# hermanjakobsen/robotic-ultrasound-imaging

Hardware: AMD Instinct MI355X
Metric: env-steps/sec (whole node) at 4096 envs/GPU, random-action rollout (higher is better)
Workload: dtype f32

## Files before the change

### robotic-ultrasound-imaging_amd/csrc/usim_api.hip

```cpp
#include <hip/hip_runtime.h>
#include <cstdio>
#include <cstdlib>
#include <cstring>
#include <string>
#include <vector>
#include <new>

#include "../../include/usim.h"
#include "usim_device.h"
#include "usim_robot.h"
#include "usim_setup.h"
#include "usim_checkpoint.h"
#include "usim_kernels.hip"
#include "usim_snapshot.h"


using namespace usim;

enum class Launch : int { STEP, MULTI, ACTS, RESET };
constexpr Launch launch_kind(bool reset, int nsub, int substeps, const float* act) {
    return reset ? Launch::RESET : nsub > 1 ? (act ? Launch::ACTS : Launch::MULTI) : substeps > 1 ? Launch::MULTI : Launch::STEP;
}

using StepKernel = void (*)(const DevModel, const DevCfg, float*, int, int, const DevIO, int, long long);
using SplitKernel = void (*)(const DevModel*, const DevCfg*, float*, int, int, const DevIO, int, long long);
struct Kernel { StepKernel step; SplitKernel split; int epb, nt, lds_words; };
struct Row { Mapping map; bool warm; Launch launch; Kernel k; };

template <Launch L> constexpr Row full_row() {
    static_assert(L == Launch::STEP || L == Launch::RESET, "the full torso runs one step per launch");
    StepKernel f = nullptr;
    if constexpr (L == Launch::STEP) f = usim_step_kernel<2, 64, 0>;
    else f = usim_step_kernel<2, 64, 1>;
    return {Mapping::FULL, false, L, {f, nullptr, FULL_EPB, FULL_NT, FULL_LDS_WORDS}};
}
template <int TORSO, int OCC, bool WARM, Launch L> constexpr Row wave_row() {
    static_assert((TORSO == 1 || (TORSO == 0 && OCC == 2 && !WARM)) && (L != Launch::RESET || OCC == 2), "RIGID16, SOFT16_W1, SOFT16_W2; resets with the budget of two waves per SIMD");
    StepKernel f = nullptr;
    if constexpr (L == Launch::STEP) f = usim_step16_kernel<TORSO, OCC, 0, false, WARM>;
    else if constexpr (L == Launch::MULTI) f = usim_step16_kernel<TORSO, OCC, 0, true, WARM>;
    else if constexpr (L == Launch::ACTS) f = usim_step16_acts_kernel<TORSO, OCC, WARM>;
    else f = usim_step16_kernel<TORSO, OCC, 1, false, WARM>;
    return {TORSO == 0 ? Mapping::RIGID16 : OCC == 1 ? Mapping::SOFT16_W1 : Mapping::SOFT16_W2, WARM, L, {f, nullptr, 16, 256, arm_lds_base<TORSO, 0, 16>() + ARM_LDS_WORDS}};
}
template <int G, bool WARM, Launch L> constexpr Row split_row() {
    static_assert((G == 16 || G == 8) && L != Launch::RESET, "SPLIT16, SPLIT8; they reset with SOFT16_W2's kernel");
    SplitKernel f = nullptr;
    if constexpr (L == Launch::STEP) f = usim_step32_kernel<false, G, WARM>;
    else if constexpr (L == Launch::MULTI) f = usim_step32_kernel<true, G, WARM>;
    else f = usim_step32_acts_kernel<G, WARM>;
    return {G == 16 ? Mapping::SPLIT16 : Mapping::SPLIT8, WARM, L, {nullptr, f, (64 / G) * SPLIT_WPR, 128 * SPLIT_WPR, arm_lds_base<1, 1, G>() + ARM_LDS_WORDS}};
}

constexpr Row kRows[] = {
    wave_row<0, 2, false, Launch::ACTS>(),
    wave_row<1, 1, true, Launch::ACTS>(), wave_row<1, 1, false, Launch::ACTS>(), wave_row<1, 2, true, Launch::ACTS>(), wave_row<1, 2, false, Launch::ACTS>(),
    split_row<16, true, Launch::ACTS>(), split_row<16, false, Launch::ACTS>(), split_row<8, true, Launch::ACTS>(), split_row<8, false, Launch::ACTS>(),

    wave_row<1, 2, true, Launch::RESET>(),
    wave_row<1, 1, true, Launch::MULTI>(), wave_row<1, 1, true, Launch::STEP>(), wave_row<1, 2, true, Launch::MULTI>(), wave_row<1, 2, true, Launch::STEP>(),
    split_row<16, true, Launch::MULTI>(), split_row<16, true, Launch::STEP>(), split_row<8, true, Launch::MULTI>(), split_row<8, true, Launch::STEP>(),

    full_row<Launch::RESET>(), full_row<Launch::STEP>(),
    wave_row<0, 2, false, Launch::MULTI>(), wave_row<0, 2, false, Launch::STEP>(), wave_row<0, 2, false, Launch::RESET>(),
    wave_row<1, 1, false, Launch::MULTI>(), wave_row<1, 1, false, Launch::STEP>(), wave_row<1, 2, false, Launch::MULTI>(), wave_row<1, 2, false, Launch::STEP>(),
    wave_row<1, 2, false, Launch::RESET>(),
    split_row<16, false, Launch::MULTI>(), split_row<16, false, Launch::STEP>(), split_row<8, false, Launch::MULTI>(), split_row<8, false, Launch::STEP>(),
};

constexpr int find_row(Mapping m, bool warm, Launch l) {
    if (m == Mapping::FULL && l != Launch::RESET) l = Launch::STEP;
    if (soft_torso(m) && l == Launch::RESET) m = Mapping::SOFT16_W2;
    warm = warm && soft_torso(m);
    int at = -1, hits = 0;
    for (int i = 0; i < (int)(sizeof kRows / sizeof kRows[0]); ++i)
        if (kRows[i].map == m && kRows[i].warm == warm && kRows[i].launch == l) { at = i; ++hits; }
    return hits == 1 ? at : -1;
}
constexpr bool table_sound() {
    for (const Row& r : kRows) if (r.k.lds_words * (int)sizeof(float) > 160 * 1024 || r.k.nt > 1024 || r.k.epb < 1 || (r.k.step == nullptr) == (r.k.split == nullptr)) return false;
    for (int m = 0; m <= (int)Mapping::SPLIT8; ++m) for (int w = 0; w < 2; ++w) for (int l = 0; l <= (int)Launch::RESET; ++l) if (find_row((Mapping)m, w != 0, (Launch)l) < 0) return false;
    return true;
}
static_assert(table_sound(), "every row within 160 KB of LDS and 1024 threads; every (mapping, warm, launch) has exactly one row");
static const Kernel& kernel_of(Mapping m, bool warm, Launch l) { return kRows[find_row(m, warm, l)].k; }

struct usim_handle {
    usim_config cfg;
    Mapping map = Mapping::RIGID16;
    StateLayout L{};
    int device = 0, adim = 6;
    DevModel M;
    DevCfg C;
    float* state = nullptr;
    float* d_tables = nullptr;
    void* d_consts = nullptr;
    const DevModel* d_M = nullptr; const DevCfg* d_C = nullptr;
    hipEvent_t ev0 = nullptr, ev1 = nullptr;
    static constexpr int RF_RING = 8;
    hipEvent_t rf0[RF_RING] = {}, rf1[RF_RING] = {};
    bool rf_live[RF_RING] = {};
    int rf_next = 0;
    double rf_total_ms = 0.0;
    long long rf_count = 0;
// ... 429 lines not shown
```

### robotic-ultrasound-imaging_amd/csrc/usim_step16.h

```cpp
#pragma once
#include <type_traits>

namespace usim {

template <int N, class F>
DI void static_for(F&& f) {
    if constexpr (N > 0) { static_for<N - 1>(f); f(std::integral_constant<int, N - 1>{}); }
}

template <int CTRL>
DI float dpp0(float v) { return __int_as_float(__builtin_amdgcn_update_dpp(0, __float_as_int(v), CTRL, 0xf, 0xf, true)); }
template <int G> DI int glane() { return (int)(threadIdx.x & (G - 1)); }
template <int G, int K> DI float rbc(float v) {
    if constexpr (G == 16) return dpp0<0x150 + K>(v);
    else {
        const int iv = __float_as_int(v);
        const int t = __builtin_amdgcn_update_dpp(iv, iv, 0x150 + K, 0xf, 0x3, false);
        return __int_as_float(__builtin_amdgcn_update_dpp(t, iv, 0x150 + 8 + K, 0xf, 0xc, false));
    }
}
template <int G, int D> DI float rshr0(float v) {
    const float t = dpp0<0x110 + D>(v);
    if constexpr (G == 16) return t; else return (glane<G>() < D) ? 0.f : t;
}
// ... 110 lines not shown
DI void fk16(const float* at, const float q, f3& X, f3& Y, f3& Z, f3& P) {
    float s, c;
    sincos_(q, s, c);
    const f3 f0 = mk(at[AT_RFIX], at[AT_RFIX + 1], at[AT_RFIX + 2]), f1 = mk(at[AT_RFIX + 3], at[AT_RFIX + 4], at[AT_RFIX + 5]);
    X = f0 * c + f1 * s; Y = f1 * c - f0 * s; Z = mk(at[AT_RFIX + 6], at[AT_RFIX + 7], at[AT_RFIX + 8]);
    P = mk(at[AT_LPOS], at[AT_LPOS + 1], at[AT_LPOS + 2]);
    static_for<3>([&](auto Dc) {
        constexpr int D = 1 << decltype(Dc)::value;
        const f3 LX = mk(rshr<G, D>(X.x, 1.f), rshr<G, D>(X.y, 0.f), rshr<G, D>(X.z, 0.f));
        const f3 LY = mk(rshr<G, D>(Y.x, 0.f), rshr<G, D>(Y.y, 1.f), rshr<G, D>(Y.z, 0.f));
        const f3 LZ = mk(rshr<G, D>(Z.x, 0.f), rshr<G, D>(Z.y, 0.f), rshr<G, D>(Z.z, 1.f));
        const f3 LP = mk(rshr0<G, D>(P.x), rshr0<G, D>(P.y), rshr0<G, D>(P.z));
        const f3 nX = LX * X.x + LY * X.y + LZ * X.z, nY = LX * Y.x + LY * Y.y + LZ * Y.z, nZ = LX * Z.x + LY * Z.y + LZ * Z.z;
        P = LP + LX * P.x + LY * P.y + LZ * P.z;
        X = nX; Y = nY; Z = nZ;
    });
}

DI void jacobian_rows(float* xl, const int gl, const float* Jc, float* Jr) {
    if (gl < 8) {
#pragma unroll
        for (int a = 0; a < 6; ++a) xl[a * 8 + gl] = Jc[a];
    }
    group_sync();
    int arow = (gl & 7) - ((gl & 4) ? 1 : 0);
    arow = arow > 5 ? 5 : arow;
    const float4 j0 = *reinterpret_cast<const float4*>(&xl[arow * 8]), j1 = *reinterpret_cast<const float4*>(&xl[arow * 8 + 4]);
    Jr[0] = j0.x; Jr[1] = j0.y; Jr[2] = j0.z; Jr[3] = j0.w; Jr[4] = j1.x; Jr[5] = j1.y; Jr[6] = j1.z; Jr[7] = j1.w;
}

template <int G>
DI float solve6_task(float* A, float b, const int gl) {
    static_for<6>([&](auto Kc) {
        constexpr int k = decltype(Kc)::value;
        constexpr int lk = TASK_LANE[k];
        const float g = (A[k] - (gl == lk ? 1.f : 0.f)) * rcp_(rbc<G, lk>(A[k]));
#pragma unroll
        for (int c = k + 1; c < 6; ++c) A[c] = fmaf(-g, rbc<G, lk>(A[c]), A[c]);
        b = fmaf(-g, rbc<G, lk>(b), b);
    });
    return b;
}

constexpr int X16_WORDS = 64;
constexpr int X16_RIGID_STRIDE = 84;

constexpr int SPLIT_WPR = 4;
constexpr int MB_POSE = X16_WORDS;
constexpr int MB_OP = MB_POSE + 12;
constexpr int MB_W = MB_OP + 64;
constexpr int MB_Q = MB_W + 16;
constexpr int MB_GOAL = MB_Q + 100;
constexpr int MB_ACT = MB_GOAL + 12;
constexpr int X2_STRIDE = MB_ACT + 8;
template <int G> constexpr int x2_base() { return TB_WORDS + (64 * SPLIT_WPR / G) * GE_STRIDE; }
static_assert(x2_base<16>() % 4 == 0 && x2_base<8>() % 4 == 0 && X2_STRIDE % 4 == 0 && MB_OP % 4 == 0 && MB_W % 4 == 0 && MB_ACT % 4 == 0, "mailbox block: 16-byte accesses");
static_assert((x2_base<8>() + 32 * X2_STRIDE) * 4 <= 160 * 1024, "split kernel with 8-lane groups: LDS of a CU");
template <int G> constexpr int arm_cull_rounds() { return G == 16 ? 0 : 7; }
template <int ROLE, int G, bool RES> constexpr bool lattice_ahead() { return ROLE != 0 && G == 16 && RES; }

#if defined(USIM_TSTAMP) || defined(USIM_TSTAMP_NOWAIT)
#define USIM_BAR() do { __syncthreads(); ++nbar; } while (0)
#else
#define USIM_BAR() __syncthreads()
#endif


constexpr int ARM_LDS_WORDS = A16_LANES * AT_STRIDE;
template <int TORSO, int ROLE, int G> constexpr int arm_lds_base();
template <int NE, class WR = NoWarm>
struct Carry {
    float dqj, qdj, q0j;
    Episode ep;
    float s[NE], sd[NE];
    WR wr;
};

template <int TORSO, int ROLE, int G> constexpr int arm_lds_base() {
    return ROLE != 0 ? x2_base<G>() + (64 * SPLIT_WPR / G) * X2_STRIDE : (TORSO ? SOFT16_LDS_WORDS : 16 * X16_RIGID_STRIDE);
}
static_assert((arm_lds_base<1, 1, 8>() + ARM_LDS_WORDS) * 4 <= 160 * 1024 && arm_lds_base<1, 1, 8>() % 4 == 0 && arm_lds_base<1, 1, 16>() % 4 == 0 && arm_lds_base<1, 0, 16>() % 4 == 0
              && arm_lds_base<0, 0, 16>() % 4 == 0, "arm table behind the LDS blocks of every 16-lane kernel");

template <int NT, int G, bool RES, class WR>
DI void lattice_pass(float* lds, const DevModel& M, const DevCfg& C, float* __restrict__ st, const int n, const int npad, const DevIO& io,
                     const bool first_pass, const int sub, const bool more, int& nbar, Carry<(N_TOP + G - 1) / G, WR>& cy) {
    constexpr bool WARM = !std::is_same<WR, NoWarm>::value;
    constexpr int WPR = SPLIT_WPR, EPW = 64 / G, EPB = WPR * EPW;
    constexpr unsigned GMASK = (G == 16) ? 0xffffu : 0xffu;
    constexpr int NE = (N_TOP + G - 1) / G;
    constexpr bool LA = lattice_ahead<2, G, RES>();
    const int lane = threadIdx.x & 63, wave = (threadIdx.x >> 6) & (WPR - 1);
    const bool fresh = !RES || first_pass;
    const int gl = lane & (G - 1), ge = lane / G;
    const int gbase = lane - gl;
    const int eb = wave * EPW + ge;
    unsigned long long* const dbg = io.dbg;
    const int env = blockIdx.x * EPB + eb;
    const bool valid = env < n;
    const bool store = valid && gl == 0;
    const int ei = valid ? env : n - 1;
#define LAT(w) st[(size_t)F_LAT * npad + (size_t)ei * LAT_ENV_WORDS + (w)]
#define EB(off) lds[TB_WORDS + eb * GE_STRIDE + (off)]
    float* const warm_rows = st + warm_index(io.bank_row0, npad, (size_t)ei);
    int mbo = x2_base<G>() + eb * X2_STRIDE;
    asm volatile("" : "+v"(mbo));

    float* const xl = &lds[mbo];
    float* const goal_lds = xl + MB_GOAL;
    float at[AT_STRIDE];
    {
        constexpr int ARM_LDS = arm_lds_base<1, 2, G>();
        const float4* ap = fresh ? reinterpret_cast<const float4*>(M.tables + TB_ARM + gl * AT_STRIDE) : reinterpret_cast<const float4*>(lds + ARM_LDS + gl * AT_STRIDE);
        if (fresh) {
#pragma unroll
            for (int v = 0; v < AT_STRIDE / 4; ++v) { const float4 x = ap[v]; at[4 * v] = x.x; at[4 * v + 1] = x.y; at[4 * v + 2] = x.z; at[4 * v + 3] = x.w; }
        } else {
            const float4* lp = reinterpret_cast<const float4*>(lds + ARM_LDS + gl * AT_STRIDE);
#pragma unroll
            for (int v = 0; v < AT_STRIDE / 4; ++v) { const float4 x = lp[v]; at[4 * v] = x.x; at[4 * v + 1] = x.y; at[4 * v + 2] = x.z; at[4 * v + 3] = x.w; }
        }
    }
    const float* const sp = st + scalar_index(0, (size_t)ei);
    const bool jlane = at[AT_JOINT] != 0.f;
    const int jl = jlane ? gl : NJ - 1;
    float &dqj = cy.dqj, &qdj = cy.qdj, &q0j = cy.q0j;
    Episode& E = cy.ep;
    f3 &ts = E.ts, &te = E.te;
    float &u0 = E.u0, &vbar = E.vbar, &fzbar = E.fzbar, &fzprev = E.fzprev, &dfz = E.dfz, &kst = E.kst, &kdmp = E.kdmp, &mu = E.mu, &epret = E.epret;
    int &t = E.t, &touched = E.touched, &episode = E.episode, &status = E.status;
    float (&s_pre)[NE] = cy.s, (&sd_pre)[NE] = cy.sd;
    auto adopt = [&](const float4 nx) {
        kst = nx.x; kdmp = nx.y; mu = nx.z; t = 0;
#pragma unroll
        for (int i = 0; i < NE; ++i) { s_pre[i] = 0.f; sd_pre[i] = 0.f; }
        warm_clear(cy.wr);
    };
    if (fresh) {
        dqj = sp[F_Q + jl]; qdj = sp[F_QD + jl]; q0j = sp[F_Q0 + jl];
        float sv[20];
        {
            const float4* s4 = reinterpret_cast<const float4*>(sp + 20);
#pragma unroll
            for (int v = 0; v < 5; ++v) { const float4 x = s4[v]; sv[4 * v] = x.x; sv[4 * v + 1] = x.y; sv[4 * v + 2] = x.z; sv[4 * v + 3] = x.w; }
        }
#define SV(f) sv[(f) - 20]
        ts = mk(SV(F_TS), SV(F_TS + 1), SV(F_TS + 2)); te = mk(SV(F_TE), SV(F_TE + 1), SV(F_TE + 2));
        u0 = SV(F_U0); vbar = SV(F_VBAR); fzbar = SV(F_FZBAR); fzprev = SV(F_FZPREV); dfz = SV(F_DFZ);
        kst = SV(F_KST); kdmp = SV(F_KDMP); mu = SV(F_MU); epret = SV(F_EPRET);
        t = __float_as_int(SV(F_T)); touched = __float_as_int(SV(F_TOUCH)); episode = __float_as_int(SV(F_EPISODE)); status = __float_as_int(SV(F_STATUS));
#undef SV
#pragma unroll
        for (int i = 0; i < NE; ++i) {
            const int e = gl + i * G;
            s_pre[i] = 0.f; sd_pre[i] = 0.f;
            if (e < N_TOP) { s_pre[i] = LAT(LAT_S + e); sd_pre[i] = LAT(LAT_SD + e); }
        }
        if constexpr (WARM) warm_load(warm_rows, gl, cy.wr);
    } else if constexpr (RES && !LA) {
        const float4 nx = *reinterpret_cast<const float4*>(&lds[mbo + MB_W]);
        if (nx.w != 0.f) adopt(nx);
    }
    if (!jlane) { dqj = 0.f; qdj = 0.f; q0j = 0.f; }
    float qj = q0j + dqj;
    if (first_pass) {
// ... 136 lines not shown
    RSTAMP(6);
#if defined(USIM_TSTAMP) || defined(USIM_TSTAMP_NOWAIT)
    if (more && dbg && blockIdx.x == 0 && (threadIdx.x & (64 * WPR - 1)) == 0) dbg[62] = __builtin_readcyclecounter();
#endif
    {
        float acc_e[NE];
#pragma unroll
        for (int i = 0; i < NE; ++i) { const int e = gl + i * G; acc_e[i] = (e < N_TOP) ? EB(GE_A + e) : 0.f; }
#pragma unroll
        for (int k = 0; k < MAXC; ++k) {
#pragma unroll
            for (int i = 0; i < NE; ++i) {
                const int e = (gl + i * G < N_TOP) ? gl + i * G : N_TOP - 1;
                acc_e[i] = fmaf(lds[TB_LINV + e * LROW + cel[k]], gf[k], acc_e[i]);
            }
        }
#pragma unroll
        for (int i = 0; i < NE; ++i) {
            const int e = gl + i * G;
            if (e >= N_TOP) continue;
            const float sdn = sd_pre[i] + dt * acc_e[i];
            const float sn = s_pre[i] + dt * sdn;
            if (valid) { LAT(LAT_SD + e) = sdn; LAT(LAT_S + e) = sn; }
            if constexpr (RES) { sd_pre[i] = sdn; s_pre[i] = sn; EB(GE_S + e) = sn; }
        }
        if constexpr (WARM) { if (valid) warm_store(warm_rows, gl, cy.wr); }
    }
    RSTAMP(7);
    if (!LA || !more) USIM_BAR();
    RSTAMP(8);
#undef RSTAMP
#undef XSTAMP
#undef LAT
#undef EB
}

template <int TORSO, int MODE, int ROLE, int NT, int G = 16, bool RES = false, class WR = NoWarm, bool AHEAD = false>
DI void step16_one(float* lds, const DevModel& M, const DevCfg& C, float* __restrict__ st, const int n, const int npad, const DevIO& io, const int flags, const long long rstep,
                   const bool first_pass, const int sub, const bool more, int& nbar, Carry<TORSO ? (N_TOP + G - 1) / G : 1, WR>& cy) {
    static_assert(ROLE != 2, "the lattice / contact wave of the split kernel runs lattice_pass");
    static_assert(!AHEAD || (ROLE == 1 && RES), "action drawn ahead: the arm wave of a resident split launch");
    constexpr bool WARM = !std::is_same<WR, NoWarm>::value;
    static_assert(!WARM || (TORSO == 1 && ROLE == 0) || (TORSO == 1 && MODE == 0), "warm start: the soft-torso kernels");
    constexpr int WPR = (ROLE != 0) ? SPLIT_WPR : 4;
    constexpr int EPW = 64 / G, EPB = WPR * EPW;
    static_assert(!RES || MODE == 0, "resident state: step launches only");
    constexpr int X2_BASE = x2_base<G>();
    constexpr unsigned GMASK = (G == 16) ? 0xffffu : 0xffu;
    static_assert(G == 16 || (TORSO == 1 && MODE == 0 && ROLE != 0), "8-lane groups: the split soft-torso step only");
    constexpr int NE = TORSO ? (N_TOP + G - 1) / G : 1;
    static_assert(ROLE == 0 || (TORSO == 1 && MODE == 0), "the split kernel is the soft-torso step");
    const int lane = threadIdx.x & 63, wave = (threadIdx.x >> 6) & (WPR - 1);
    constexpr bool LA = lattice_ahead<ROLE, G, RES>();
    const bool fresh = !RES || first_pass;
    const int gl = lane & (G - 1), ge = lane / G;
    const int gbase = lane - gl;
    const int eb = wave * EPW + ge;
    const bool auto_reset = (flags & LF_AUTO_RESET) != 0;
    unsigned long long* const dbg = io.dbg;
    const bool refill = (MODE == 1) && io.refill != 0;
    const int item_cnt = refill ? io.count[0] : 1;
    const int item_first = refill ? (int)blockIdx.x * EPB : 0;
    for (int item0 = item_first; item0 < item_cnt; item0 += refill ? (int)gridDim.x * EPB : 1) {
    int env = blockIdx.x * EPB + eb;
    bool valid = env < n;
    int item_ep = 0;
    if (refill) {
        valid = item0 + eb < item_cnt;
        const int2 it = valid ? io.items[item0 + eb] : make_int2(0, 0);
        env = it.x; item_ep = it.y;
    }
    const bool store = valid && gl == 0;
    const int ei = valid ? env : (refill ? 0 : n - 1);
#define LAT(w) st[(size_t)F_LAT * npad + (size_t)ei * LAT_ENV_WORDS + (w)]
#define EB(off) lds[TB_WORDS + eb * GE_STRIDE + (off)]
    float* const warm_rows = st + warm_index(io.bank_row0, npad, (size_t)ei);
    int mbo = X2_BASE + eb * X2_STRIDE;
    if constexpr (ROLE != 0) asm volatile("" : "+v"(mbo));
    float* const xl = (ROLE != 0) ? &lds[mbo]
                                  : (TORSO ? &lds[TB_WORDS + eb * GE_STRIDE + GE_WS] : &lds[eb * X16_RIGID_STRIDE]);
    static_assert(GE_WS + X16_WORDS <= GE_STRIDE, "transpose scratch overlays the wrench records");
    constexpr int GOAL_OFF = (ROLE != 0) ? MB_GOAL : (TORSO ? GE_CG + (MAXCAND + 1) * CG_WORDS - GE_WS : X16_WORDS);
    static_assert(GE_CG + (MAXCAND + 1) * CG_WORDS + 12 <= GE_STRIDE && X16_WORDS + 12 <= X16_RIGID_STRIDE, "room for the goal");
    float* const goal_lds = xl + GOAL_OFF;

    USIM_STAMP(dbg, 0);
    if constexpr (ROLE == 1) { if (dbg && blockIdx.x == 0 && threadIdx.x == 0) dbg[20] = __builtin_readcyclecounter(); }

    float at[AT_STRIDE];
    {
        constexpr int ARM_LDS = arm_lds_base<TORSO, ROLE, G>();
        const float4* ap = fresh ? reinterpret_cast<const float4*>(M.tables + TB_ARM + gl * AT_STRIDE) : reinterpret_cast<const float4*>(lds + ARM_LDS + gl * AT_STRIDE);
        if (fresh) {
#pragma unroll
            for (int v = 0; v < AT_STRIDE / 4; ++v) { const float4 x = ap[v]; at[4 * v] = x.x; at[4 * v + 1] = x.y; at[4 * v + 2] = x.z; at[4 * v + 3] = x.w; }
            if constexpr (RES) {
                if (lane < G) {
#pragma unroll
                    for (int v = 0; v < AT_STRIDE / 4; ++v) reinterpret_cast<float4*>(lds + ARM_LDS + gl * AT_STRIDE)[v] = make_float4(at[4 * v], at[4 * v + 1], at[4 * v + 2], at[4 * v + 3]);
                }
            }
        } else {
            const float4* lp = reinterpret_cast<const float4*>(lds + ARM_LDS + gl * AT_STRIDE);
#pragma unroll
            for (int v = 0; v < AT_STRIDE / 4; ++v) { const float4 x = lp[v]; at[4 * v] = x.x; at[4 * v + 1] = x.y; at[4 * v + 2] = x.z; at[4 * v + 3] = x.w; }
        }
    }
    const float* const sp = st + scalar_index(0, (size_t)ei);
    const bool jlane = at[AT_JOINT] != 0.f;
    const int jl = jlane ? gl : NJ - 1;
    float &dqj = cy.dqj, &qdj = cy.qdj, &q0j = cy.q0j;
    Episode& E = cy.ep;
    f3 &ts = E.ts, &te = E.te;
    float &u0 = E.u0, &vbar = E.vbar, &fzbar = E.fzbar, &fzprev = E.fzprev, &dfz = E.dfz, &kst = E.kst, &kdmp = E.kdmp, &mu = E.mu, &epret = E.epret;
    int &t = E.t, &touched = E.touched, &episode = E.episode, &status = E.status;
    float (&s_pre)[NE] = cy.s, (&sd_pre)[NE] = cy.sd;
    if (fresh) {
        dqj = sp[F_Q + jl]; qdj = sp[F_QD + jl]; q0j = sp[F_Q0 + jl];
        float sv[20];
        {
            const float4* s4 = reinterpret_cast<const float4*>(sp + 20);
#pragma unroll
            for (int v = 0; v < 5; ++v) { const float4 x = s4[v]; sv[4 * v] = x.x; sv[4 * v + 1] = x.y; sv[4 * v + 2] = x.z; sv[4 * v + 3] = x.w; }
        }
#define SV(f) sv[(f) - 20]
        ts = mk(SV(F_TS), SV(F_TS + 1), SV(F_TS + 2)); te = mk(SV(F_TE), SV(F_TE + 1), SV(F_TE + 2));
        u0 = SV(F_U0); vbar = SV(F_VBAR); fzbar = SV(F_FZBAR); fzprev = SV(F_FZPREV); dfz = SV(F_DFZ);
        kst = SV(F_KST); kdmp = SV(F_KDMP); mu = SV(F_MU); epret = SV(F_EPRET);
        t = __float_as_int(SV(F_T)); touched = __float_as_int(SV(F_TOUCH)); episode = __float_as_int(SV(F_EPISODE)); status = __float_as_int(SV(F_STATUS));
#undef SV
#pragma unroll
        for (int i = 0; i < NE; ++i) {
            const int e = gl + i * G;
            s_pre[i] = 0.f; sd_pre[i] = 0.f;
            if (TORSO && MODE == 0 && ROLE == 0 && e < N_TOP) { s_pre[i] = LAT(LAT_S + e); sd_pre[i] = LAT(LAT_SD + e); }
            if (TORSO && MODE == 0 && ROLE == 1 && !LA && e < N_TOP) s_pre[i] = LAT(LAT_S + e);
        }
        if constexpr (WARM && MODE == 0 && ROLE == 0) warm_load(warm_rows, gl, cy.wr);
    } else if constexpr (RES && ROLE == 1 && !LA) {
#pragma unroll
        for (int i = 0; i < NE; ++i) { const int e = gl + i * G; s_pre[i] = (e < N_TOP) ? EB(GE_S + e) : 0.f; }
    }
    if (!jlane) { dqj = 0.f; qdj = 0.f; q0j = 0.f; }
    float qj = q0j + dqj;
// ... 350 lines not shown
    const float alpha_t = row_times_joint<G, NJ>(Jr, qs);
    f3 s_rc, s_wwrc, s_nw, s_arm, s_xso;
    float qe[4], obs[OBS_DIM], pos_err_norm = 0.f, pos_rew = 0.f, ori_err = 0.f, ori_rew = 0.f, vel_rew = 0.f, force_e = 0.f, dforce_e = 0.f;
    f3 xw, tpw;
    auto rot_inertia = [&](f3 v) {
        const f3 l = mk(dot(X, v), dot(Y, v), dot(Z, v));
        const f3 tt = symmul(M.pI7, l);
        return X * tt.x + Y * tt.y + Z * tt.z;
    };
    auto precompute = [&]() {
        s_rc = X * M.pcom7[0] + Y * M.pcom7[1] + Z * M.pcom7[2];
        s_wwrc = cross(w, cross(w, s_rc));
        s_nw = cross(w, rot_inertia(w));
        s_xso = xs - P;
        s_arm = s_rc - s_xso;
        const int tprev = (MODE == 0) ? t - 1 : 0;
        const float up = clampf((float)tprev * inv_h + u0, 0.f, 1.f);
        tpw = ts + (te - ts) * up;
        xw = mk(xs.x + M.base[0], xs.y + M.base[1], xs.z + M.base[2]);
        obs[12] = xw.x - tpw.x; obs[13] = xw.y - tpw.y; obs[14] = xw.z - tpw.z;
        mat2quat_xyzw(sx, sy, sz, qe);
        difference_quat(qe, M.gquat, obs + 15);
        if constexpr (MODE == 0) {
            float pe0 = 90.f * (xw.x - tpw.x), pe1 = 90.f * (xw.y - tpw.y);
            pe0 *= pe0; pe1 *= pe1;
            pos_err_norm = sqrt_(pe0 * pe0 + pe1 * pe1);
            pos_rew = 5.f * exp_(-pos_err_norm);
            const float qc[4] = {qe[3], qe[0], qe[1], qe[2]};
            ori_err = 0.2f * distance_quat_goal(qc, M.ghat, M.geps);
            ori_rew = exp_(-ori_err);
            float ve = 45.f * (vbar - 0.04f); ve *= ve;
            vel_rew = exp_(-ve);
            float fe = 0.7f * (fzbar - 5.f); fe *= fe;
            force_e = 3.f * exp_(-fe);
            float de = 0.01f * dfz; de *= de;
            dforce_e = 2.f * exp_(-de);
        }
    };
    float W[6] = {0, 0, 0, 0, 0, 0};
    int ncon = 0, overflow = 0, con_shell[MAXC];
#pragma unroll
    for (int k = 0; k < MAXC; ++k) con_shell[k] = -1;
    if constexpr (ROLE == 1) {
        if (is_task) {
            const int arow = blk ? 3 + comp : comp;
            float* mbo = xl + MB_OP;
            *reinterpret_cast<float4*>(&mbo[arow * 8]) = make_float4(Li[0], Li[1], Li[2], Li[3]);
            mbo[arow * 8 + 4] = Li[4]; mbo[arow * 8 + 5] = Li[5];
            mbo[48 + arow] = alpha_t; mbo[54 + arow] = v6;
        }
        RSTAMP(3);
        USIM_BAR();
        RSTAMP(4);
        precompute();
        if constexpr (AHEAD) {
            if ((flags & LF_RANDOM_ACT) && more && last_sub) {
                float nxt[7];
                draw_action(rstep + 1, nxt);
                keep_action(nxt);
            }
        }
        RSTAMP(5);
        USIM_BAR();
        RSTAMP(6);
#if defined(USIM_TSTAMP) || defined(USIM_TSTAMP_NOWAIT)
        if (more && dbg && blockIdx.x == 0 && (threadIdx.x & (64 * WPR - 1)) == 0) dbg[63] = __builtin_readcyclecounter();
#endif
        const float4 w0 = *reinterpret_cast<const float4*>(&xl[MB_W]), w1 = *reinterpret_cast<const float4*>(&xl[MB_W + 4]);
        W[0] = w0.x; W[1] = w0.y; W[2] = w0.z; W[3] = w0.w; W[4] = w1.x; W[5] = w1.y;
        ncon = __float_as_int(w1.z); overflow = __float_as_int(w1.w);
        if (io.contacts) {
            const int* tb_shell = reinterpret_cast<const int*>(lds + TB_SHELL);
            const float4 e0 = *reinterpret_cast<const float4*>(&xl[MB_W + 8]), e1 = *reinterpret_cast<const float4*>(&xl[MB_W + 12]);
            const int el[MAXC] = {__float_as_int(e0.x), __float_as_int(e0.y), __float_as_int(e0.z), __float_as_int(e0.w),
                                  __float_as_int(e1.x), __float_as_int(e1.y), __float_as_int(e1.z), __float_as_int(e1.w)};
#pragma unroll
            for (int k = 0; k < MAXC; ++k) { const int sh = tb_shell[el[k]]; con_shell[k] = (k < ncon) ? sh : -1; }
        }
    } else if constexpr (TORSO != 0) {
        const int* tb_shell = reinterpret_cast<const int*>(lds + TB_SHELL);
        float dz, vz, az;
        torso_motion(C, tphys, dz, vz, az);
        lattice_rhs<G, NE>(lds, eb, gl, M, az, kst, kdmp, MODE == 0, s_pre, sd_pre);
        USIM_STAMP(dbg, 5);
        int nc = collide_all<G, NE>(lds, eb, gl, gbase, M, C, MODE == 0, s_pre, dz, xs, sy, sz);
        lattice_solve<G>(lds, eb, gl, gbase);
        contact_overflow<G>(lds, eb, gl, gbase, nc);
        USIM_STAMP(dbg, 7);
        if (nc > MAXC) { overflow = 1; nc = MAXC; }
        ncon = nc;
        group_sync();
        int ncmax = 0;
#pragma unroll
        for (int k = MAXC; k >= 1; --k) if (ncmax == 0 && __any(nc >= k)) ncmax = k;
        float gf[MAXC];
        int cel[MAXC];
#pragma unroll
        for (int k = 0; k < MAXC; ++k) { gf[k] = 0.f; cel[k] = (k < nc) ? __float_as_int(EB(GE_CG + k * CG_WORDS + 6)) : 0; }
        if (ncmax > 0) {
            float alpha[6], vs[6], Lp[21];
            static_for<6>([&](auto Ac) {
                constexpr int a = decltype(Ac)::value;
                alpha[a] = rbc<G, TASK_LANE[a]>(alpha_t); vs[a] = rbc<G, TASK_LANE[a]>(v6);
#pragma unroll
                for (int b = 0; b <= a; ++b) Lp[PK(a, b)] = rbc<G, TASK_LANE[a]>(Li[b]);
            });
            USIM_STAMP(dbg, 8);
            if constexpr (MODE == 0) contact_solve<G, false, false>(lds, eb, gl, M, C, nc, ncmax, cel, Lp, alpha, vs, mu, vz, ContactRows{}, W, gf, dbg, cy.wr);
            else { NoWarm cold; contact_solve<G, false, false>(lds, eb, gl, M, C, nc, ncmax, cel, Lp, alpha, vs, mu, vz, ContactRows{}, W, gf, dbg, cold); }
        } else warm_clear(cy.wr);
        USIM_STAMP(dbg, 11);
        if constexpr (MODE == 1) {
            if (valid && need && !refill) {
                for (int e = gl; e < N_TOP; e += G) { LAT(LAT_S + e) = 0.f; LAT(LAT_SD + e) = 0.f; }
                if constexpr (WARM) warm_rows_clear<G>(warm_rows, gl);
            }
        } else {
            float acc_e[NE];
#pragma unroll
            for (int i = 0; i < NE; ++i) { const int e = gl + i * G; acc_e[i] = (e < N_TOP) ? EB(GE_A + e) : 0.f; }
#pragma unroll
            for (int k = 0; k < MAXC; ++k) {
                if (k < ncmax) {
#pragma unroll
                    for (int i = 0; i < NE; ++i) {
                        const int e = (gl + i * G < N_TOP) ? gl + i * G : N_TOP - 1;
                        acc_e[i] = fmaf(lds[TB_LINV + e * LROW + cel[k]], gf[k], acc_e[i]);
                    }
                }
            }
#pragma unroll
            for (int i = 0; i < NE; ++i) {
                const int e = gl + i * G;
                if (e >= N_TOP) continue;
                const float sdn = sd_pre[i] + dt * acc_e[i];
                const float sn = s_pre[i] + dt * sdn;
                if (valid) { LAT(LAT_SD + e) = sdn; LAT(LAT_S + e) = sn; }
                if constexpr (RES) { sd_pre[i] = sdn; s_pre[i] = sn; }
            }
            if constexpr (WARM) { if (valid) warm_store(warm_rows, gl, cy.wr); }
        }
#pragma unroll
        for (int k = 0; k < MAXC; ++k) con_shell[k] = (k < nc) ? tb_shell[cel[k]] : -1;
    }
    USIM_STAMP(dbg, 12);

    if constexpr (ROLE != 1) precompute();
    float tq[3];
    f3 hv;
    {
        float qacc = qs, aq_t = alpha_t;
        if (TORSO) {
#pragma unroll
            for (int a = 0; a < 6; ++a) { qacc = fmaf(Xm[a], W[a], qacc); aq_t = fmaf(Li[a], W[a], aq_t); }
        }
        float aq[6];
        static_for<6>([&](auto Ac) { constexpr int a = decltype(Ac)::value; aq[a] = rbc<G, TASK_LANE[a]>(aq_t); });
        const f3 alq = mk(aq[3], aq[4], aq[5]);
        const f3 alt = al + alq;
        const f3 a7 = ao + mk(aq[0], aq[1], aq[2]) - cross(alq, s_xso);
        const f3 ac = a7 + cross(alt, s_rc) + s_wwrc;
        const f3 N = rot_inertia(alt) + s_nw;
        const f3 Fp = ac * PROBE_MASS;
        const f3 tw = N + cross(s_arm, Fp) - mk(W[3], W[4], W[5]);
        tq[0] = rbc<G, NJ - 1>(dot(sx, tw)); tq[1] = rbc<G, NJ - 1>(dot(sy, tw)); tq[2] = rbc<G, NJ - 1>(dot(sz, tw));
        USIM_STAMP(dbg, 13);
        hv = mk(0, 0, 0);
        if constexpr (MODE == 0) {
            const float xk = row_times_joint<G, NJ>(Mi, qacc);
            const float rhs = fmaf(-dt * JOINT_DAMP, xk, qacc);
            qdj = fmaf(dt, rhs, qdj); dqj = fmaf(dt, qdj, dqj);
            if (!jlane) { qdj = 0.f; dqj = 0.f; }
            qj = q0j + dqj;
            const float v2_t = row_times_joint<G, NJ>(Jr, qdj);
            float v2[6];
            static_for<6>([&](auto Ac) { constexpr int a = decltype(Ac)::value; v2[a] = rbc<G, TASK_LANE[a]>(v2_t); });
            hv = mk(v2[0], v2[1], v2[2]) + cross(mk(v2[3], v2[4], v2[5]), hand - xs);
        }
    }
    USIM_STAMP(dbg, 14);

    bool done = false;
    {
        if (MODE == 1) fzbar = W[2];
        obs[0] = W[0]; obs[1] = W[1]; obs[2] = W[2];
        obs[3] = tq[0]; obs[4] = tq[1]; obs[5] = tq[2];
        obs[6] = hv.x; obs[7] = hv.y; obs[8] = hv.z;
        obs[9] = fzbar - 5.0f; obs[10] = dfz - 0.0f; obs[11] = vbar - 0.04f;
        if constexpr (MODE == 1) {
            if (overflow) status |= 1;
            if (refill) {
                if (valid && need) {
                    const int sl = ep_t & (BANK_DEPTH - 1);
                    if (jlane) BK(sl, BQ0 + gl) = qj;
                    if (gl == 0) {
                        BK(sl, BTS) = ts.x; BK(sl, BTS + 1) = ts.y; BK(sl, BTS + 2) = ts.z; BK(sl, BTE) = te.x; BK(sl, BTE + 1) = te.y; BK(sl, BTE + 2) = te.z;
                        BK(sl, BU0) = u0; BK(sl, BKST) = kst; BK(sl, BKDMP) = kdmp; BK(sl, BMU) = mu; BK(sl, BFZ) = fzbar;
#pragma unroll
                        for (int a = 0; a < OBS_DIM; ++a) BK(sl, BOBS + a) = obs[a];
                        BKI(sl, BSTATUS) = overflow ? 1 : 0;
                    }
                }
            } else if (store && io.obs && need) {
#pragma unroll
                for (int a = 0; a < OBS_DIM; ++a) io.obs[(size_t)ei * OBS_DIM + a] = obs[a];
            }
        } else if (last_sub) {
        const bool contact = ncon > 0;
        if (contact) touched = 1;
        const float force_rew = contact ? force_e : 0.f, dforce_rew = contact ? dforce_e : 0.f;
        float reward = pos_rew + ori_rew + vel_rew + force_rew + dforce_rew;
        done = t >= C.horizon;
        const float hvn = sqrt_(dot(hv, hv));
        vbar += (hvn - vbar) * rcp_((float)t);
        const float fz = W[2];
        dfz = (fz - fzprev) * rcp_(C.dt_ctrl);
        fzprev = fz;
        fzbar = 0.1f * fz + 0.9f * fzbar;
        const bool jviol = (qj < at[AT_QMIN] + 0.1f) || (qj > at[AT_QMAX] - 0.1f);
        const unsigned jany = (unsigned)(__ballot(jviol) >> gbase) & GMASK;
        if (C.early_term) {
            const bool term = (jany != 0u) || (pos_err_norm > 1.0f) || (contact && ori_err > 0.10f) || (touched && !contact);
            done = done || term;
        }
        epret += reward;
        if (io.log && valid) {
            float* L = io.log + (size_t)ei * LOG_WIDTH;
            if (jlane) L[26 + gl] = qj;
            if (gl == 0) {
                const float upn = clampf((float)t * inv_h + u0, 0.f, 1.f);
                const f3 tpn = ts + (te - ts) * upn;
                L[0] = xw.x; L[1] = xw.y; L[2] = xw.z; L[3] = tpn.x; L[4] = tpn.y; L[5] = tpn.z;
                L[6] = hv.x; L[7] = hv.y; L[8] = hv.z; L[9] = 0.04f; L[10] = vbar;
                L[11] = qe[0]; L[12] = qe[1]; L[13] = qe[2]; L[14] = qe[3];
                L[15] = M.gquat[0]; L[16] = M.gquat[1]; L[17] = M.gquat[2]; L[18] = M.gquat[3];
                L[19] = ori_err * 5.0f;
                L[20] = fz; L[21] = 5.0f; L[22] = fzbar; L[23] = dfz; L[24] = 0.f; L[25] = contact ? 1.f : 0.f;
                L[40] = (float)(t - 1) * inv_h * 100.f;
                L[41] = pos_rew; L[42] = ori_rew; L[43] = vel_rew; L[44] = force_rew; L[45] = dforce_rew;
            }
        }
        if (overflow) status |= 1;
        {
            const float chk = rbc<G, 7>(prefix_sum<G>(fabsf(qj) + 1e-3f * fabsf(qdj)));
            if (!(chk < 1.0e3f)) { status |= 4; done = true; epret -= reward; reward = 0.f; if (!(epret == epret)) epret = 0.f; }
        }
        if (store) {
            io.rew[ei] = reward;
            if (io.status_out) io.status_out[ei] = status;
            io.done[ei] = done ? 1 : 0;
            if (io.contacts) {
                io.contacts[(size_t)ei * (1 + MAXC)] = ncon;
#pragma unroll
                for (int k = 0; k < MAXC; ++k) io.contacts[(size_t)ei * (1 + MAXC) + 1 + k] = con_shell[k];
            }
            if (done) {
                if (io.term_obs) {
#pragma unroll
                    for (int a = 0; a < OBS_DIM; ++a) io.term_obs[(size_t)ei * OBS_DIM + a] = obs[a];
                }
                if (io.ep_ret) io.ep_ret[ei] = epret;
                if (io.ep_len) io.ep_len[ei] = t;
            }
        }
        need = done && auto_reset;
        if (store && io.obs && !need) {
#pragma unroll
            for (int a = 0; a < OBS_DIM; ++a) io.obs[(size_t)ei * OBS_DIM + a] = obs[a];
        }
        }
    }

    if constexpr (ROLE == 1) { RSTAMP(7); if (!LA || !more) USIM_BAR(); RSTAMP(8); }
    if (MODE == 0 && need) {
        episode += 1;
        const int sl = episode & (BANK_DEPTH - 1);
        qj = jlane ? BK(sl, BQ0 + jl) : 0.f; q0j = qj; qdj = 0.f; dqj = 0.f;
        ts = mk(BK(sl, BTS), BK(sl, BTS + 1), BK(sl, BTS + 2)); te = mk(BK(sl, BTE), BK(sl, BTE + 1), BK(sl, BTE + 2));
        u0 = BK(sl, BU0); kst = BK(sl, BKST); kdmp = BK(sl, BKDMP); mu = BK(sl, BMU); fzbar = BK(sl, BFZ);
        episode_begin(E, BKI(sl, BSTATUS));
        if (store && io.obs) {
#pragma unroll
            for (int a = 0; a < OBS_DIM; ++a) io.obs[(size_t)ei * OBS_DIM + a] = BK(sl, BOBS + a);
        }
        const bool zero_here = !LA || !more;
        if (TORSO && valid && zero_here) for (int e = gl; e < N_TOP; e += G) { LAT(LAT_S + e) = 0.f; LAT(LAT_SD + e) = 0.f; }
        if constexpr (WARM) {
            if (valid && zero_here) warm_rows_clear<G>(warm_rows, gl);
            warm_clear(cy.wr);
        }
        if constexpr (RES && TORSO != 0) {
#pragma unroll
            for (int i = 0; i < NE; ++i) {
                s_pre[i] = 0.f; sd_pre[i] = 0.f;
                if (ROLE == 1 && !LA && gl + i * G < N_TOP) EB(GE_S + gl + i * G) = 0.f;
            }
        }
        if (store) order_refill(io, env, episode);
    }
    if constexpr (RES && ROLE == 1) {
        if (gl == 0) *reinterpret_cast<float4*>(&xl[MB_W]) = make_float4(kst, kdmp, mu, (MODE == 0 && need) ? 1.f : 0.f);
    }
    USIM_STAMP(dbg, 15);

    if (valid && (MODE == 0 || (need && !refill))) {
        float* const so = st + scalar_index(0, (size_t)ei);
        if (jlane) {
            so[F_Q + gl] = dqj; so[F_QD + gl] = qdj;
            if (need) so[F_Q0 + gl] = q0j;
        }
        if (gl == 0) {
            float4* s4 = reinterpret_cast<float4*>(so);
            if (need) {
                so[F_TS] = ts.x; so[F_TS + 1] = ts.y; so[F_TS + 2] = ts.z;
                s4[6] = make_float4(te.x, te.y, te.z, u0);
            }
            s4[7] = make_float4(vbar, fzbar, fzprev, dfz);
            s4[8] = make_float4(kst, kdmp, mu, __int_as_float(t));
            s4[9] = make_float4(__int_as_float(touched), __int_as_float(episode), epret, __int_as_float(status));
        }
    }
    if (refill) group_sync();
    }
    if (MODE == 1 && refill) work_list_close(io);
    USIM_STAMP(dbg, 16);
    if constexpr (ROLE == 1) RSTAMP(9);
#undef RSTAMP
#undef LAT
#undef EB
}

template <int TORSO, int MODE, int ROLE, int NT, bool MULTI = false, int G = 16, class WR = NoWarm, bool ACTS = false>
DI void step16_body(float* lds, const DevModel& M, const DevCfg& C, float* __restrict__ st, const int n, const int npad, const DevIO& io0, const int flags, const long long rstep) {
    const int S = (MULTI && MODE == 0 && C.substeps > 1) ? C.substeps : 1;
    const int nsub = (MULTI && MODE == 0) ? (io0.nsub > 1 ? io0.nsub : 1) * S : 1;
    DevIO io = io0;
    int nbar = 0;
    Carry<TORSO ? (N_TOP + G - 1) / G : 1, WR> cy;
    int sub = 0;
    long long cstep = rstep;
    for (int ks = 0; ks < nsub; ++ks) {
        constexpr bool AHEAD = ROLE == 1 && MULTI && MODE == 0 && !ACTS;
        if constexpr (ROLE == 2) lattice_pass<NT, G, MULTI && MODE == 0, WR>(lds, M, C, st, n, npad, io, ks == 0, sub, ks + 1 < nsub, nbar, cy);
        else step16_one<TORSO, MODE, ROLE, NT, G, MULTI && MODE == 0, WR, AHEAD>(lds, M, C, st, n, npad, io, flags, cstep, ks == 0, sub, ks + 1 < nsub, nbar, cy);
        const bool ctrl_done = sub == S - 1;
        if (ctrl_done) { sub = 0; ++cstep; } else ++sub;
        if (ks + 1 < nsub) {
            constexpr bool LA = lattice_ahead<ROLE, G, MULTI && MODE == 0>();
            if constexpr (!LA) {
                __threadfence_block();
                if constexpr (ROLE != 0) USIM_BAR();
            }
            if (io0.block && ctrl_done) advance_rollout_block(io, (size_t)n, C.adim);
            if constexpr (ACTS) { if (ctrl_done) io.act += (size_t)n * C.adim; }
        }
    }
#if defined(USIM_TSTAMP) || defined(USIM_TSTAMP_NOWAIT)
    if (ROLE != 0 && io0.dbg && blockIdx.x == 0 && (threadIdx.x & (64 * SPLIT_WPR - 1)) == 0) io0.dbg[ROLE == 1 ? 46 : 47] = (unsigned long long)nbar;
// ... 41 lines not shown
```

Baseline: 254.2 million.

## Defer split-kernel step reporting to the next pass via LDS report mailbox

In the 16-lane split kernel with resident multi-step launches, the end-of-step torque/observation finish and the global writes of reward, done, obs, contacts and scalar state are deferred. The needed intermediates go into a new per-env LDS report area, and the next pass completes the computation and stores them after its barrier. This takes the cross-lane broadcasts and global stores off the critical path at the end of each step and overlaps them with the next step's precompute. In exchange it uses more LDS per env, which can reduce occupancy, and adds complex bookkeeping for block-offset output pointers and reset handling.

```diff
diff --git a/robotic-ultrasound-imaging_amd/csrc/usim_api.hip b/robotic-ultrasound-imaging_amd/csrc/usim_api.hip
--- a/robotic-ultrasound-imaging_amd/csrc/usim_api.hip
+++ b/robotic-ultrasound-imaging_amd/csrc/usim_api.hip
@@ -49,7 +49,7 @@
     if constexpr (L == Launch::STEP) f = usim_step32_kernel<false, G, WARM>;
     else if constexpr (L == Launch::MULTI) f = usim_step32_kernel<true, G, WARM>;
     else f = usim_step32_acts_kernel<G, WARM>;
-    return {G == 16 ? Mapping::SPLIT16 : Mapping::SPLIT8, WARM, L, {nullptr, f, (64 / G) * SPLIT_WPR, 128 * SPLIT_WPR, arm_lds_base<1, 1, G>() + ARM_LDS_WORDS}};
+    return {G == 16 ? Mapping::SPLIT16 : Mapping::SPLIT8, WARM, L, {nullptr, f, (64 / G) * SPLIT_WPR, 128 * SPLIT_WPR, arm_lds_base<1, 1, G, L != Launch::STEP>() + ARM_LDS_WORDS}};
 }
 
 constexpr Row kRows[] = {
diff --git a/robotic-ultrasound-imaging_amd/csrc/usim_step16.h b/robotic-ultrasound-imaging_amd/csrc/usim_step16.h
--- a/robotic-ultrasound-imaging_amd/csrc/usim_step16.h
+++ b/robotic-ultrasound-imaging_amd/csrc/usim_step16.h
@@ -186,10 +186,20 @@
 constexpr int MB_Q = MB_W + 16;
 constexpr int MB_GOAL = MB_Q + 100;
 constexpr int MB_ACT = MB_GOAL + 12;
-constexpr int X2_STRIDE = MB_ACT + 8;
+constexpr int MB_REP = MB_ACT + 8;
+constexpr int REP_LINK = 0;
+constexpr int REP_SITE = 32;
+constexpr int REP_W = 52;
+constexpr int REP_SHELL = 68;
+constexpr int REP_AQ = 76;
+constexpr int REP_WORDS = 84;
+template <int G, bool RES> constexpr bool report_late() { return G == 16 && RES; }
+template <bool REP> constexpr int x2_stride() { return MB_REP + (REP ? REP_WORDS : 0); }
 template <int G> constexpr int x2_base() { return TB_WORDS + (64 * SPLIT_WPR / G) * GE_STRIDE; }
-static_assert(x2_base<16>() % 4 == 0 && x2_base<8>() % 4 == 0 && X2_STRIDE % 4 == 0 && MB_OP % 4 == 0 && MB_W % 4 == 0 && MB_ACT % 4 == 0, "mailbox block: 16-byte accesses");
-static_assert((x2_base<8>() + 32 * X2_STRIDE) * 4 <= 160 * 1024, "split kernel with 8-lane groups: LDS of a CU");
+static_assert(x2_base<16>() % 4 == 0 && x2_base<8>() % 4 == 0 && x2_stride<false>() % 4 == 0 && x2_stride<true>() % 4 == 0 && MB_OP % 4 == 0 && MB_W % 4 == 0 && MB_ACT % 4 == 0
+              && MB_REP % 4 == 0 && REP_SITE % 4 == 0 && REP_W % 4 == 0 && REP_SHELL % 4 == 0 && REP_AQ % 4 == 0 && REP_WORDS % 4 == 0, "mailbox block: 16-byte accesses");
+static_assert((x2_base<8>() + 32 * x2_stride<false>()) * 4 <= 160 * 1024, "split kernel with 8-lane groups: LDS of a CU");
+static_assert(OBS_DIM == 19 && MAXC == 8 && REP_AQ + 8 == REP_WORDS, "layout of the report area");
 template <int G> constexpr int arm_cull_rounds() { return G == 16 ? 0 : 7; }
 template <int ROLE, int G, bool RES> constexpr bool lattice_ahead() { return ROLE != 0 && G == 16 && RES; }
 
@@ -201,7 +211,7 @@
 
 
 constexpr int ARM_LDS_WORDS = A16_LANES * AT_STRIDE;
-template <int TORSO, int ROLE, int G> constexpr int arm_lds_base();
+template <int TORSO, int ROLE, int G, bool RES = false> constexpr int arm_lds_base();
 template <int NE, class WR = NoWarm>
 struct Carry {
     float dqj, qdj, q0j;
@@ -210,11 +220,12 @@
     WR wr;
 };
 
-template <int TORSO, int ROLE, int G> constexpr int arm_lds_base() {
-    return ROLE != 0 ? x2_base<G>() + (64 * SPLIT_WPR / G) * X2_STRIDE : (TORSO ? SOFT16_LDS_WORDS : 16 * X16_RIGID_STRIDE);
+template <int TORSO, int ROLE, int G, bool RES> constexpr int arm_lds_base() {
+    return ROLE != 0 ? x2_base<G>() + (64 * SPLIT_WPR / G) * x2_stride<report_late<G, RES>()>() : (TORSO ? SOFT16_LDS_WORDS : 16 * X16_RIGID_STRIDE);
 }
 static_assert((arm_lds_base<1, 1, 8>() + ARM_LDS_WORDS) * 4 <= 160 * 1024 && arm_lds_base<1, 1, 8>() % 4 == 0 && arm_lds_base<1, 1, 16>() % 4 == 0 && arm_lds_base<1, 0, 16>() % 4 == 0
-              && arm_lds_base<0, 0, 16>() % 4 == 0, "arm table behind the LDS blocks of every 16-lane kernel");
+              && arm_lds_base<0, 0, 16>() % 4 == 0 && arm_lds_base<1, 1, 16, true>() % 4 == 0 && arm_lds_base<1, 1, 8, true>() == arm_lds_base<1, 1, 8>()
+              && (arm_lds_base<1, 1, 16, true>() + ARM_LDS_WORDS) * 4 <= 160 * 1024, "arm table behind the LDS blocks of every 16-lane kernel");
 
 template <int NT, int G, bool RES, class WR>
 DI void lattice_pass(float* lds, const DevModel& M, const DevCfg& C, float* __restrict__ st, const int n, const int npad, const DevIO& io,
@@ -237,14 +248,14 @@
 #define LAT(w) st[(size_t)F_LAT * npad + (size_t)ei * LAT_ENV_WORDS + (w)]
 #define EB(off) lds[TB_WORDS + eb * GE_STRIDE + (off)]
     float* const warm_rows = st + warm_index(io.bank_row0, npad, (size_t)ei);
-    int mbo = x2_base<G>() + eb * X2_STRIDE;
+    int mbo = x2_base<G>() + eb * x2_stride<report_late<G, RES>()>();
     asm volatile("" : "+v"(mbo));
 
     float* const xl = &lds[mbo];
     float* const goal_lds = xl + MB_GOAL;
     float at[AT_STRIDE];
     {
-        constexpr int ARM_LDS = arm_lds_base<1, 2, G>();
+        constexpr int ARM_LDS = arm_lds_base<1, 2, G, RES>();
         const float4* ap = fresh ? reinterpret_cast<const float4*>(M.tables + TB_ARM + gl * AT_STRIDE) : reinterpret_cast<const float4*>(lds + ARM_LDS + gl * AT_STRIDE);
         if (fresh) {
 #pragma unroll
@@ -487,6 +498,8 @@
     static_assert(ROLE == 0 || (TORSO == 1 && MODE == 0), "the split kernel is the soft-torso step");
     const int lane = threadIdx.x & 63, wave = (threadIdx.x >> 6) & (WPR - 1);
     constexpr bool LA = lattice_ahead<ROLE, G, RES>();
+    constexpr bool DEF = ROLE == 1 && report_late<G, RES>();
+    const bool defer = DEF && more;
     const bool fresh = !RES || first_pass;
     const int gl = lane & (G - 1), ge = lane / G;
     const int gbase = lane - gl;
@@ -510,7 +523,7 @@
 #define LAT(w) st[(size_t)F_LAT * npad + (size_t)ei * LAT_ENV_WORDS + (w)]
 #define EB(off) lds[TB_WORDS + eb * GE_STRIDE + (off)]
     float* const warm_rows = st + warm_index(io.bank_row0, npad, (size_t)ei);
-    int mbo = X2_BASE + eb * X2_STRIDE;
+    int mbo = X2_BASE + eb * x2_stride<ROLE != 0 && report_late<G, RES>()>();
     if constexpr (ROLE != 0) asm volatile("" : "+v"(mbo));
     float* const xl = (ROLE != 0) ? &lds[mbo]
                                   : (TORSO ? &lds[TB_WORDS + eb * GE_STRIDE + GE_WS] : &lds[eb * X16_RIGID_STRIDE]);
@@ -524,7 +537,7 @@
 
     float at[AT_STRIDE];
     {
-        constexpr int ARM_LDS = arm_lds_base<TORSO, ROLE, G>();
+        constexpr int ARM_LDS = arm_lds_base<TORSO, ROLE, G, RES>();
         const float4* ap = fresh ? reinterpret_cast<const float4*>(M.tables + TB_ARM + gl * AT_STRIDE) : reinterpret_cast<const float4*>(lds + ARM_LDS + gl * AT_STRIDE);
         if (fresh) {
 #pragma unroll
@@ -981,7 +994,114 @@
         RSTAMP(3);
         USIM_BAR();
         RSTAMP(4);
+        if constexpr (DEF) {
+            if (!first_pass) {
+                const float* const rp = xl + MB_REP;
+                const bool tr = sub == 0;
+                const float4* const wk = reinterpret_cast<const float4*>(&rp[REP_W]);
+                const float4 w0 = wk[0], w1 = wk[1], w2 = wk[2], w3 = wk[3];
+                const int pflags = tr ? __float_as_int(w3.y) : 0;
+                const bool pdone = (pflags & 1) != 0, pneed = (pflags & 2) != 0;
+                if (tr) {
+                    float* p_obs = io.obs; float* p_rew = io.rew; uint8_t* p_done = io.done; float* p_term = io.term_obs; int* p_con = io.contacts;
+                    float* p_ret = io.ep_ret; int* p_len = io.ep_len;
+                    if (io.block) {
+                        const size_t rows = (size_t)n;
+                        p_obs -= rows * OBS_DIM; p_rew -= rows; p_done -= rows;
+                        if (p_term) p_term -= rows * OBS_DIM;
+                        if (p_con) p_con -= rows * (1 + MAXC);
+                        if (p_ret) p_ret -= rows;
+                        if (p_len) p_len -= rows;
+                    }
+                    const float4* const lk = reinterpret_cast<const float4*>(&rp[REP_LINK]);
+                    const float4 k0 = lk[0], k1 = lk[1], k2 = lk[2], k3 = lk[3], k4 = lk[4], k5 = lk[5], k6 = lk[6], k7 = lk[7];
+                    const f3 p_al = mk(k0.x, k0.y, k0.z), p_ao = mk(k0.w, k1.x, k1.y), p_xso = mk(k1.z, k1.w, k2.x), p_rc = mk(k2.y, k2.z, k2.w), p_wwrc = mk(k3.x, k3.y, k3.z);
+                    const f3 p_nw = mk(k3.w, k4.x, k4.y), p_arm = mk(k4.z, k4.w, k5.x), pX = mk(k5.y, k5.z, k5.w), pY = mk(k6.x, k6.y, k6.z), pZ = mk(k6.w, k7.x, k7.y);
+                    const float4* const sk = reinterpret_cast<const float4*>(&rp[REP_SITE]);
+                    const float4 s0 = sk[0], s1 = sk[1], s2 = sk[2], s3 = sk[3], s4 = sk[4];
+                    const f3 p_sx = mk(s0.x, s0.y, s0.z), p_sy = mk(s0.w, s1.x, s1.y), p_sz = mk(s1.z, s1.w, s2.x);
+                    const float4 q0 = *reinterpret_cast<const float4*>(&rp[REP_AQ]), q1 = *reinterpret_cast<const float4*>(&rp[REP_AQ + 4]);
+                    const f3 alq = mk(q0.w, q1.x, q1.y);
+                    const f3 alt = p_al + alq;
+                    const f3 a7 = p_ao + mk(q0.x, q0.y, q0.z) - cross(alq, p_xso);
+                    const f3 ac = a7 + cross(alt, p_rc) + p_wwrc;
+                    const f3 il = mk(dot(pX, alt), dot(pY, alt), dot(pZ, alt));
+                    const f3 it = symmul(M.pI7, il);
+                    const f3 N = (pX * it.x + pY * it.y + pZ * it.z) + p_nw;
+                    const f3 Fp = ac * PROBE_MASS;
+                    const f3 tw = N + cross(p_arm, Fp) - mk(w0.w, w1.x, w1.y);
+                    const float po[OBS_DIM] = {w0.x, w0.y, w0.z, dot(p_sx, tw), dot(p_sy, tw), dot(p_sz, tw), w1.z, w1.w, w2.x, s2.y, s2.z, s2.w,
+                                               s3.x, s3.y, s3.z, s3.w, s4.x, s4.y, s4.z};
+                    if (store) {
+                        p_rew[ei] = w2.y;
+                        if (io.status_out) io.status_out[ei] = __float_as_int(w3.x);
+                        p_done[ei] = pdone ? 1 : 0;
+                        if (p_con) {
+                            const float4 h0 = *reinterpret_cast<const float4*>(&rp[REP_SHELL]), h1 = *reinterpret_cast<const float4*>(&rp[REP_SHELL + 4]);
+                            const int sh[MAXC] = {__float_as_int(h0.x), __float_as_int(h0.y), __float_as_int(h0.z), __float_as_int(h0.w),
+                                                  __float_as_int(h1.x), __float_as_int(h1.y), __float_as_int(h1.z), __float_as_int(h1.w)};
+                            p_con[(size_t)ei * (1 + MAXC)] = __float_as_int(w3.z);
+#pragma unroll
+                            for (int k = 0; k < MAXC; ++k) p_con[(size_t)ei * (1 + MAXC) + 1 + k] = sh[k];
+                        }
+                        if (pdone) {
+                            if (p_term) {
+#pragma unroll
+                                for (int a = 0; a < OBS_DIM; ++a) p_term[(size_t)ei * OBS_DIM + a] = po[a];
+                            }
+                            if (p_ret) p_ret[ei] = w2.z;
+                            if (p_len) p_len[ei] = __float_as_int(w2.w);
+                        }
+                        if (p_obs) {
+                            if (!pneed) {
+#pragma unroll
+                                for (int a = 0; a < OBS_DIM; ++a) p_obs[(size_t)ei * OBS_DIM + a] = po[a];
+                            } else {
+                                const int sl = episode & (BANK_DEPTH - 1);
+#pragma unroll
+                                for (int a = 0; a < OBS_DIM; ++a) p_obs[(size_t)ei * OBS_DIM + a] = BK(sl, BOBS + a);
+                            }
+                        }
+                    }
+                }
+                if (valid) {
+                    float* const so = st + scalar_index(0, (size_t)ei);
+                    if (jlane) {
+                        so[F_Q + gl] = dqj; so[F_QD + gl] = qdj;
+                        if (pneed) so[F_Q0 + gl] = q0j;
+                    }
+                    if (gl == 0) {
+                        float4* s4 = reinterpret_cast<float4*>(so);
+                        if (pneed) {
+                            so[F_TS] = ts.x; so[F_TS + 1] = ts.y; so[F_TS + 2] = ts.z;
+                            s4[6] = make_float4(te.x, te.y, te.z, u0);
+                        }
+                        s4[7] = make_float4(vbar, fzbar, fzprev, dfz);
+                        s4[8] = make_float4(kst, kdmp, mu, __int_as_float(tr ? t - 1 : t));
+                        s4[9] = make_float4(__int_as_float(touched), __int_as_float(episode), epret, __int_as_float(status));
+                    }
+                }
+                RSTAMP(29);
+            }
+        }
         precompute();
+        if constexpr (DEF) {
+            if (defer && last_sub) {
+                float* const rp = xl + MB_REP;
+                if (gl == NJ - 1) {
+                    float4* const lk = reinterpret_cast<float4*>(&rp[REP_LINK]);
+                    lk[0] = make_float4(al.x, al.y, al.z, ao.x); lk[1] = make_float4(ao.y, ao.z, s_xso.x, s_xso.y); lk[2] = make_float4(s_xso.z, s_rc.x, s_rc.y, s_rc.z);
+                    lk[3] = make_float4(s_wwrc.x, s_wwrc.y, s_wwrc.z, s_nw.x); lk[4] = make_float4(s_nw.y, s_nw.z, s_arm.x, s_arm.y); lk[5] = make_float4(s_arm.z, X.x, X.y, X.z);
+                    lk[6] = make_float4(Y.x, Y.y, Y.z, Z.x); lk[7] = make_float4(Z.y, Z.z, 0.f, 0.f);
+                }
+                if (gl == 0) {
+                    float4* const sk = reinterpret_cast<float4*>(&rp[REP_SITE]);
+                    sk[0] = make_float4(sx.x, sx.y, sx.z, sy.x); sk[1] = make_float4(sy.y, sy.z, sz.x, sz.y);
+                    sk[2] = make_float4(sz.z, fzbar - 5.0f, dfz - 0.0f, vbar - 0.04f);
+                    sk[3] = make_float4(obs[12], obs[13], obs[14], obs[15]); sk[4] = make_float4(obs[16], obs[17], obs[18], 0.f);
+                }
+            }
+        }
         if constexpr (AHEAD) {
             if ((flags & LF_RANDOM_ACT) && more && last_sub) {
                 float nxt[7];
@@ -1083,6 +1203,7 @@
 #pragma unroll
             for (int a = 0; a < 6; ++a) { qacc = fmaf(Xm[a], W[a], qacc); aq_t = fmaf(Li[a], W[a], aq_t); }
         }
+        if (!defer) {
         float aq[6];
         static_for<6>([&](auto Ac) { constexpr int a = decltype(Ac)::value; aq[a] = rbc<G, TASK_LANE[a]>(aq_t); });
         const f3 alq = mk(aq[3], aq[4], aq[5]);
@@ -1093,6 +1214,10 @@
         const f3 Fp = ac * PROBE_MASS;
         const f3 tw = N + cross(s_arm, Fp) - mk(W[3], W[4], W[5]);
         tq[0] = rbc<G, NJ - 1>(dot(sx, tw)); tq[1] = rbc<G, NJ - 1>(dot(sy, tw)); tq[2] = rbc<G, NJ - 1>(dot(sz, tw));
+        } else {
+            tq[0] = 0.f; tq[1] = 0.f; tq[2] = 0.f;
+            if (is_task) xl[MB_REP + REP_AQ + (blk ? 3 + comp : comp)] = aq_t;
+        }
         USIM_STAMP(dbg, 13);
         hv = mk(0, 0, 0);
         if constexpr (MODE == 0) {
@@ -1174,7 +1299,7 @@
             const float chk = rbc<G, 7>(prefix_sum<G>(fabsf(qj) + 1e-3f * fabsf(qdj)));
             if (!(chk < 1.0e3f)) { status |= 4; done = true; epret -= reward; reward = 0.f; if (!(epret == epret)) epret = 0.f; }
         }
-        if (store) {
+        if (store && !defer) {
             io.rew[ei] = reward;
             if (io.status_out) io.status_out[ei] = status;
             io.done[ei] = done ? 1 : 0;
@@ -1193,9 +1318,22 @@
             }
         }
         need = done && auto_reset;
-        if (store && io.obs && !need) {
+        if (store && io.obs && !need && !defer) {
 #pragma unroll
             for (int a = 0; a < OBS_DIM; ++a) io.obs[(size_t)ei * OBS_DIM + a] = obs[a];
+        }
+        if constexpr (DEF) {
+            if (defer && gl == 0) {
+                float4* const wk = reinterpret_cast<float4*>(&xl[MB_REP + REP_W]);
+                wk[0] = make_float4(W[0], W[1], W[2], W[3]); wk[1] = make_float4(W[4], W[5], hv.x, hv.y);
+                wk[2] = make_float4(hv.z, reward, epret, __int_as_float(t));
+                wk[3] = make_float4(__int_as_float(status), __int_as_float((done ? 1 : 0) | (need ? 2 : 0)), __int_as_float(ncon), 0.f);
+                if (io.contacts) {
+                    float4* const hk = reinterpret_cast<float4*>(&xl[MB_REP + REP_SHELL]);
+                    hk[0] = make_float4(__int_as_float(con_shell[0]), __int_as_float(con_shell[1]), __int_as_float(con_shell[2]), __int_as_float(con_shell[3]));
+                    hk[1] = make_float4(__int_as_float(con_shell[4]), __int_as_float(con_shell[5]), __int_as_float(con_shell[6]), __int_as_float(con_shell[7]));
+                }
+            }
         }
         }
     }
@@ -1208,7 +1346,7 @@
         ts = mk(BK(sl, BTS), BK(sl, BTS + 1), BK(sl, BTS + 2)); te = mk(BK(sl, BTE), BK(sl, BTE + 1), BK(sl, BTE + 2));
         u0 = BK(sl, BU0); kst = BK(sl, BKST); kdmp = BK(sl, BKDMP); mu = BK(sl, BMU); fzbar = BK(sl, BFZ);
         episode_begin(E, BKI(sl, BSTATUS));
-        if (store && io.obs) {
+        if (store && io.obs && !defer) {
 #pragma unroll
             for (int a = 0; a < OBS_DIM; ++a) io.obs[(size_t)ei * OBS_DIM + a] = BK(sl, BOBS + a);
         }
@@ -1231,8 +1369,9 @@
         if (gl == 0) *reinterpret_cast<float4*>(&xl[MB_W]) = make_float4(kst, kdmp, mu, (MODE == 0 && need) ? 1.f : 0.f);
     }
     USIM_STAMP(dbg, 15);
-
-    if (valid && (MODE == 0 || (need && !refill))) {
+    if constexpr (DEF) { if (more) RSTAMP(28); }
+
+    if (valid && (MODE == 0 || (need && !refill)) && !defer) {
         float* const so = st + scalar_index(0, (size_t)ei);
         if (jlane) {
             so[F_Q + gl] = dqj; so[F_QD + gl] = qdj;
```

New measurement: 257.5 million (median of 6 runs). 1.3% higher.
